# shichaoy/cube_slam

Hardware: AMD Instinct MI355X
Metric: frames/sec front-end (ORB extract + LSD+LBD lines + cuboid: Canny+DT+sweep+score+select) @640x480 (higher is better)
Workload: dtype f64

## Files before the change

cube_slam_amd/csrc/frontend.hip:

```cpp
#include "common.h"

#include <condition_variable>
#include <map>
#include <mutex>
#include <thread>
#include <vector>

extern "C" int cs_lsd_run(cs_ctx *ctx, cs_lsd *l, int with_lbd);
void cs_lsd_set_gate(cs_lsd *l, void (*wait)(void *), void (*done)(void *), void *arg);
void cs_lsd_set_shared_gpu(cs_lsd *l, int shared);
extern "C" int cs_orb_run(cs_ctx *ctx, cs_orb *e);
extern "C" int cs_cuboid_batch_run(cs_ctx *ctx, cs_cuboid_batch *b);
extern "C" int cs_cuboid_batch_set_shared_gpu(cs_cuboid_batch *b, int shared);
extern "C" int cs_cuboid_batch_set_lines(cs_ctx *ctx, cs_cuboid_batch *b, const int *line_offsets, const double *lines);
extern "C" int cs_cuboid_batch_n_frames(const cs_cuboid_batch *b);
extern "C" int cs_cuboid_batch_set_gray_device(cs_ctx *ctx, cs_cuboid_batch *b, const uint8_t *d_gray);
extern "C" int cs_cuboid_batch_set_scene(cs_ctx *ctx, cs_cuboid_batch *b, const double *Twc, const int *box_offsets, const double *boxes, const int *line_offsets, const double *lines);
extern "C" int cs_orb_set_frames_device(cs_ctx *ctx, cs_orb *e, const uint8_t *d_gray, int n_frames);
extern "C" int cs_orb_geometry(const cs_orb *e, int *width, int *height, int *max_frames);
extern "C" int cs_lsd_geometry(const cs_lsd *l, int *width, int *height, int *max_frames);
extern "C" int cs_cuboid_batch_geometry(const cs_cuboid_batch *b, int *width, int *height, int *n_frames);
extern "C" int cs_lsd_set_frames_device(cs_ctx *ctx, cs_lsd *l, const uint8_t *d_gray, int n_frames);
extern "C" int cs_orb_read_packed_on(cs_orb *e, void *stream, cs_keypoint *kps, uint8_t *desc, long cap_total, int *first, long *total);
extern "C" int cs_cuboid_batch_read_on(cs_cuboid_batch *b, void *stream, cs_cuboid *out, int *counts, int *status_out);
int cs_lsd_filter_lines_packed(cs_lsd *l, float length_thres, std::vector<int> &offsets, std::vector<double> &lines);

struct cs_frontend;
namespace {
struct LinePacket { std::vector<int> off; std::vector<double> lines; int status = CS_OK; };
struct Gate {
    std::mutex m; std::condition_variable cv;
    bool phased = false;
    long submitted = 0, target = 0, done = 0;
};
struct FrameRing {
    int n_slots = 0, n_frames = 0; size_t bytes = 0;
    hipStream_t copy = nullptr, copy_out = nullptr;
    hipEvent_t step_done = nullptr, cub_done = nullptr, results_out = nullptr; bool results_pending = false, status_read = false; int *h_status = nullptr;
    std::vector<uint8_t *> d;
    std::vector<hipEvent_t> uploaded, used_main, used_line;
    std::vector<long> main_gen, line_gen;
    struct Scene { bool has = false, has_lines = false; std::vector<double> Twc, boxes, lines; std::vector<int> box_off, line_off; };
    std::vector<Scene> scene;
    std::mutex m; std::condition_variable cv;
    long pushed = 0, first = 0, first_line = 0;
};
struct LineWorker {
    cs_ctx *ctx = nullptr; cs_lsd *lsd = nullptr;
    Gate *gate = nullptr; long ticket = 0; bool marked = true;
    static void gate_wait(void *arg) {
        LineWorker *w = (LineWorker *)arg; Gate *g = w->gate;
        std::unique_lock<std::mutex> lk(g->m);
        if (w->marked) return;
// ... 82 lines not shown
    bool may_start() const { return passes_started < passes_target && passes_started < step_no + lead_max() && (!ring || passes_started < ring->pushed); }
    void kick_idle() {
        for (size_t k = 0; k < workers.size() && may_start(); k++) {
            const size_t c = (next_worker + k) % workers.size();
            if (!workers[c]->is_free()) continue;
            workers[c]->submit(passes_started++);
            next_worker = (c + 1) % workers.size();
        }
    }
};

namespace {
int LineWorker::take_frames() {
    if (!fe || !fe->ring) return CS_OK;
    FrameRing *R = fe->ring;
    const int slot = (int)(pass_no % R->n_slots);
    if (hipSetDevice(ctx->device) != hipSuccess || hipStreamWaitEvent(ctx->stream, R->uploaded[slot], 0) != hipSuccess) return CS_ERR_HIP;
    int r = cs_lsd_set_frames_device(ctx, lsd, R->d[slot], R->n_frames);
    if (r == CS_OK && hipEventRecord(R->used_line[slot], ctx->stream) != hipSuccess) r = CS_ERR_HIP;
    { std::lock_guard<std::mutex> lk(R->m); R->line_gen[slot] = pass_no; }
    R->cv.notify_all();
    return r;
}
bool LineWorker::after_pass(int r) {
    if (!fe) return false;
    LinePacket pk; bool leave = false;
    if (fe->chain && pass_no >= fe->chain_first) {
        leave = true; pk.status = r;
        if (r == CS_OK) pk.status = cs_lsd_filter_lines_packed(lsd, fe->chain_thres, pk.off, pk.lines);
    }
    std::lock_guard<std::mutex> lk(fe->any_m);
    if (leave) { fe->packets[pass_no] = std::move(pk); fe->any_cv.notify_all(); }
    if (r != CS_OK || fe->gate.phased || !fe->may_start()) return false;
    pass_no = fe->passes_started++;
    return true;
}
}

extern "C" {

int cs_frontend_create(cs_ctx *ctx, cs_orb *orb, cs_cuboid_batch *batch, int n_line_workers, cs_ctx *const *line_ctx, cs_lsd *const *lsd, cs_frontend **out) {
    if (!ctx || !out || n_line_workers < 0 || n_line_workers > 8 || (n_line_workers && (!line_ctx || !lsd))) return CS_ERR_BAD_ARG;
    for (int i = 0; i < n_line_workers; i++) if (!line_ctx[i] || !lsd[i] || line_ctx[i] == ctx) return CS_ERR_BAD_ARG;
    cs_frontend *fe = new (std::nothrow) cs_frontend();
    if (!fe) return CS_ERR_NOMEM;
    fe->ctx = ctx; fe->orb = orb; fe->batch = batch;
    for (int i = 0; i < n_line_workers; i++) {
        LineWorker *w = new LineWorker();
        w->ctx = line_ctx[i]; w->lsd = lsd[i]; w->gate = &fe->gate; w->any_m = &fe->any_m; w->any_cv = &fe->any_cv; w->fe = fe;
        cs_lsd_set_gate(w->lsd, LineWorker::gate_wait, LineWorker::gate_done, w);
        w->th = std::thread([w] { w->loop(); });
        fe->workers.push_back(w);
    }
    fe->streams = 1 + 2 * n_line_workers;
    { const char *q = getenv("GPU_MAX_HW_QUEUES"); fe->hw_queues = q && atoi(q) > 0 ? atoi(q) : 4; }
    if (fe->hw_queues < fe->streams) {
        static bool said = false;
        if (!said) { said = true; fprintf(stderr, "[cubeslam-hip] cs_frontend_create: %d streams on %d hardware queues (GPU_MAX_HW_QUEUES%s): streams that share a queue run one after the other -- a 100 ms region walk then "
                                          "stalls another stream's kernels (up to -25 %% measured).  Export GPU_MAX_HW_QUEUES=16 before the HIP runtime starts (INTEGRATION.md).\n", fe->streams, fe->hw_queues, getenv("GPU_MAX_HW_QUEUES") ? "" : " unset: the runtime's default"); }
    }
    if (fe->batch) cs_cuboid_batch_set_shared_gpu(fe->batch, n_line_workers > 0);
    for (LineWorker *w : fe->workers) cs_lsd_set_shared_gpu(w->lsd, n_line_workers > 1);
    *out = fe;
    return CS_OK;
}

int cs_frontend_queues(const cs_frontend *fe, int *streams, int *hw_queues) {
    if (!fe) return CS_ERR_BAD_ARG;
    if (streams) *streams = fe->streams;
    if (hw_queues) *hw_queues = fe->hw_queues;
    return fe->hw_queues >= fe->streams ? 1 : 0;
}

int cs_frontend_step(cs_frontend *fe) {
    if (!fe) return CS_ERR_BAD_ARG;
    int r = CS_OK;
    if (fe->ring) {
        std::lock_guard<std::mutex> lk(fe->any_m);
        if (fe->step_no >= fe->ring->pushed) { fe->ctx->err = "cs_frontend_step: the streaming source holds no frames for this step (cs_frontend_stream_push first)"; return CS_ERR_BAD_ARG; }
    }
    if (!fe->workers.empty()) {
        const long W = (long)fe->workers.size();
        LinePacket pk; bool have_pk = false;
        {
            std::unique_lock<std::mutex> lk(fe->any_m);
            const long k = fe->step_no;
            if (fe->passes_target < k + 1) fe->passes_target = k + 1;
            if (fe->gate.phased) {
                if (fe->passes_started <= k) { LineWorker *w = fe->workers[(size_t)(k % W)]; const long no = fe->passes_started++; lk.unlock(); w->submit(no); lk.lock(); fe->in_phase++; }
            } else {
                fe->kick_idle();
                while (fe->passes_started <= k) { fe->any_cv.wait_for(lk, std::chrono::milliseconds(2)); fe->kick_idle(); }
            }
            if (fe->chain && fe->batch && k - W >= fe->chain_first) {
                fe->any_cv.wait(lk, [&] { return fe->packets.count(k - W) != 0; });
                pk = std::move(fe->packets[k - W]); fe->packets.erase(k - W); have_pk = true;
            }
            fe->step_no = k + 1;
        }
        if (have_pk) {
            r = pk.status;
            if (r == CS_OK && (long)pk.off.size() != (long)cs_cuboid_batch_n_frames(fe->batch) + 1) r = CS_ERR_BAD_ARG;
            if (r == CS_OK) r = cs_cuboid_batch_set_lines(fe->cub_ctx ? fe->cub_ctx : fe->ctx, fe->batch, pk.off.data(), pk.lines.data());
            if (r != CS_OK) return r;
        }
    } else {
        std::lock_guard<std::mutex> lk(fe->any_m);
// ... 203 lines not shown
```

cube_slam_amd/csrc/lsd_regions.h:

```cpp
#pragma once
#include <vector>

#include <hip/hip_runtime.h>
struct cs_ctx;
struct LsdSeq;
int lsd_seq_run(cs_ctx *ctx, LsdSeq **handle, int F, int w, int h, const float *d_ang, const double *d_mod, const int *d_caddr, const float *d_cdeg, const float2 *d_ccs, const int *frame_base,
                std::vector<std::vector<float>> &lines, long *stats, void (*before_seq)(void *), void (*after_seq)(void *), void *gate_arg, int grp_p, int waves_per_workgroup = 16, void *scratch = nullptr,
                size_t scratch_bytes = 0, bool pix_ready = false, bool walk_bg = false);
void lsd_seq_destroy(LsdSeq *r);
```

cube_slam_amd/csrc/lsd_regions.hip:

```cpp
#include "common.h"

#include <cfloat>
#include <climits>
#include <cmath>
#include <vector>

#include "lsd_regions.h"
#include "lsd_rg_seq.h"
#include "lsd_rg_wlk.h"

namespace {
constexpr int PAD_PX = 272, PAD_LIST = 272, PAD_RECT = 34;
constexpr double PI_ = rg::PI_, LOG_EPS = 0.0, LSD_SCALE = 0.8;
struct AngMap { int w, h; const float *deg; };

__device__ __forceinline__ double rg_log_gamma_windschitl(double x) { return 0.918938533204673 + (x - 0.5) * log(x) - x + 0.5 * x * log(x * sinh(1 / x) + 1 / (810.0 * pow(x, 6.0))); }
__device__ double rg_log_gamma(double x) {
    if (x > 15.0) return rg_log_gamma_windschitl(x);
    const double q[7] = {75122.6331530, 80916.6278952, 36308.2951477, 8687.24529705, 1168.92649479, 83.8676043424, 2.50662827511};
    double a = (x + 0.5) * log(x + 5.5) - (x + 5.5), b = 0;
    for (int n = 0; n < 7; ++n) { a -= log(x + double(n)); b += q[n] * pow(x, double(n)); }
    return a + log(b);
}
#ifndef RG_IMPROVE_WAVES
// ... 121 lines not shown
    if (log_nfa > LOG_EPS) return log_nfa;
    const int g = lane >> 3, sub = lane & 7;
    rg::Rect mine;
    int tot = 0, al = 0, cnt = 0;
    auto tolerances = [&]() {
        mine = rec;
        double p = rec.p, precs[5];
#pragma unroll
        for (int n = 0; n < 5; ++n) { p /= 2; precs[n] = p * PI_; if (n <= g) { mine.p = p; mine.prec = precs[n]; } }
        int t, alg[5]; rg_rect_count<5>(F, rec, precs, lane, t, alg);
        tot = t; al = alg[0];
#pragma unroll
        for (int n = 1; n < 5; ++n) if (g == n) al = alg[n];
        cnt = 5;
    };
    auto shrink = [&](int side) {
        mine = rec; cnt = 0;
        double wd = rec.width;
#pragma unroll
        for (int n = 0; n < 5; ++n) if ((wd - delta) >= 0.5) { wd -= delta; cnt++; }
#pragma unroll
        for (int n = 0; n < 5; ++n) if (n <= g && (mine.width - delta) >= 0.5) {
            if (side == 1) { mine.x1 += -mine.dy * delta_2; mine.y1 += mine.dx * delta_2; mine.x2 += -mine.dy * delta_2; mine.y2 += mine.dx * delta_2; }
            else if (side == 2) { mine.x1 -= -mine.dy * delta_2; mine.y1 -= mine.dx * delta_2; mine.x2 -= -mine.dy * delta_2; mine.y2 -= mine.dx * delta_2; }
            mine.width -= delta;
        }
        if (cnt) rg_rect_count_group(F, mine, g < cnt, sub, tot, al);
    };
    auto take_best = [&]() {
        const bool on = g < cnt;
        const double mv = rg_nfa(on ? tot : 0, on ? al : 0, mine.p, LOG_NT, lgt);
        int best = -1;
#pragma unroll
        for (int n = 0; n < 5; ++n) { const double vn = __shfl(mv, 8 * n); if (n < cnt && vn > log_nfa) { log_nfa = vn; best = n; } }
        if (best >= 0) rec = rg_rect_shfl(mine, 8 * best);
    };
    tolerances(); take_best();
    if (log_nfa > LOG_EPS) return log_nfa;
    for (int side = 0; side < 3; side++) {
        shrink(side);
        if (cnt) take_best();
        if (log_nfa > LOG_EPS) return log_nfa;
    }
    if ((rec.width - delta) >= 0.5) { tolerances(); take_best(); }
    return log_nfa;
}

struct SeqParams {
    int F, w, h;
    const int *caddr; const int *frame_base; const float *cdeg; const float2 *ccs; const double *mod; const float *ang;
    float *ang32; float *seed_cs; int *glist; double *rect; size_t rect_stride; int cand_cap; int *cand_cnt; int *status;
    int min_reg_size, list_cap;
    size_t pix_stride;
};
__global__ void __launch_bounds__(256) lsd_rg_fill32(float4 *ang, size_t n4) {
    const size_t i = (size_t)blockIdx.x * 256 + threadIdx.x;
    if (i < n4) ang[i] = make_float4(rgs::NOTDEF_F, rgs::NOTDEF_F, rgs::NOTDEF_F, rgs::NOTDEF_F);
}
__global__ void __launch_bounds__(256) lsd_rg_scatter(SeqParams P) {
    const int f = blockIdx.y, base = P.frame_base[f], ne = P.frame_base[f + 1] - base;
    const int i = blockIdx.x * 256 + threadIdx.x;
    if (i >= ne) return;
    const int q = P.caddr[base + i] & 0x7fffffff;
    const float d = P.cdeg[base + i];
    P.ang32[(size_t)f * P.pix_stride + q] = d;
    const double a = double(d) * rg::DEG_TO_RADS;
    reinterpret_cast<float2 *>(P.seed_cs)[base + i] = make_float2(float(cos(a)), float(sin(a)));
}
__device__ __forceinline__ void lsd_rg_seq_body(const SeqParams &P) {
    const int f = __builtin_amdgcn_readfirstlane(blockIdx.x * (blockDim.x >> 6) + (threadIdx.x >> 6));
    if (f >= P.F) return;
#ifdef RGS_PRIO
    __builtin_amdgcn_s_setprio(RGS_PRIO);
#endif
    const int base = P.frame_base[f];
    rgs::Frame Fr;
    Fr.w = P.w; Fr.h = P.h; Fr.ne = P.frame_base[f + 1] - base;
    Fr.caddr = P.caddr + base; Fr.fre = P.ang32 + (size_t)f * P.pix_stride; Fr.ang = P.ang + (size_t)f * P.w * P.h; Fr.mod = P.mod + (size_t)f * P.w * P.h; Fr.seed_cs = P.seed_cs + 2 * (size_t)base;
    Fr.rect = P.rect + (size_t)f * P.rect_stride; Fr.cand_cap = P.cand_cap; Fr.cand_cnt = P.cand_cnt + f;
    Fr.status = P.status + 4 * f; Fr.min_reg_size = P.min_reg_size; Fr.list_cap = P.list_cap;
    rgs::List L;
    L.glob = P.glist + (size_t)f * rgs::CAP; L.ring[0] = 0;
    rgs::run_frame<rgs::Wave>(Fr, L);
}
#ifdef RGS_WAVES
__global__ void __launch_bounds__(1024) __attribute__((amdgpu_waves_per_eu(RGS_WAVES, RGS_WAVES))) lsd_rg_seq(SeqParams P) { lsd_rg_seq_body(P); }
#else
__global__ void __launch_bounds__(1024) lsd_rg_seq(SeqParams P) { lsd_rg_seq_body(P); }
#endif
constexpr int WLK_SLICES = 8;
struct WlkLaunch { rgl::Batch slice[WLK_SLICES]; int n_slices, waves_per_slice; };
template <int NS> struct WlkMail {
    rgw::Mail<NS> &m; int base;
    __device__ __forceinline__ rgw::Mail<NS> &mail() { return m; }
    __device__ __forceinline__ int slot_of(int l) const { return base + l; }
    __device__ __forceinline__ int ring_size() const { return NS; }
    __device__ __forceinline__ void after_iteration(const rgl::Batch &) {}
};
template <int WK, int NWAVES, int ACC> __global__ void __launch_bounds__(64 * NWAVES) lsd_rg_wlk(WlkLaunch L, int blocks_per_slice) {
    constexpr int NS = WK * 64;
    __shared__ rgw::Mail<NS> mail;
    for (int k = threadIdx.x; k < NS; k += 64 * NWAVES) { mail.slot[k].state = 0; mail.slot[k].fl = 0; mail.ring_id[k] = 0; mail.ring_tick[k] = 0; }
    if (threadIdx.x == 0) { mail.tail = 0; mail.head = 0; mail.walkers_done = 0; }
    __syncthreads();
    const int wv = __builtin_amdgcn_readfirstlane(threadIdx.x >> 6), lane = threadIdx.x & 63;
    const int c = blockIdx.x / blocks_per_slice;
    const rgl::Batch &B = L.slice[c];
    if (wv < WK) {
        const int f0 = ((blockIdx.x - c * blocks_per_slice) * WK + wv) * 64;
        if (f0 < B.F) { WlkMail<NS> mp{mail, wv * 64}; rgw::run_walker<rgl::LWave, ACC>(B, f0, mp); }
        rgw::wg_release();
        if (lane == 0) rgw::lds_add(&mail.walkers_done, 1);
        return;
    }
    for (;;) {
        int t = 0;
        if (lane == 0) t = rgw::lds_add(&mail.head, 1);
        t = __builtin_amdgcn_readfirstlane(t);
        bool quit = false;
        while (__builtin_amdgcn_readfirstlane(rgw::lds_ld(&mail.ring_tick[t % NS])) != t + 1) {
            if (__builtin_amdgcn_readfirstlane(rgw::lds_ld(&mail.walkers_done)) == WK && __builtin_amdgcn_readfirstlane(rgw::lds_ld(&mail.tail)) <= t) { quit = true; break; }
            __builtin_amdgcn_s_sleep(4);
        }
        if (quit) break;
        rgw::serve_ticket<rgs::Wave, NS>(B, mail, t);
    }
}
__global__ void __launch_bounds__(1024) lsd_rg_cand_scan(const int *cand_cnt, int F, int *cand_base) {
    __shared__ int part[1024];
    const int t = threadIdx.x, per = (F + 1023) / 1024;
    int sum = 0;
    for (int k = 0; k < per; k++) { const int f = t * per + k; if (f < F) sum += cand_cnt[f]; }
    part[t] = sum;
    __syncthreads();
    for (int d = 1; d < 1024; d <<= 1) { const int v = t >= d ? part[t - d] : 0; __syncthreads(); part[t] += v; __syncthreads(); }
    int run = part[t] - sum;
    for (int k = 0; k < per; k++) { const int f = t * per + k; if (f < F) { cand_base[f] = run; run += cand_cnt[f]; } }
    if (t == 1023) cand_base[F] = part[1023];
}
__global__ void __launch_bounds__(256) __attribute__((amdgpu_waves_per_eu(RG_IMPROVE_WAVES, RG_IMPROVE_WAVES))) lsd_rg_improve(SeqParams P, const int *cand_base, int n_cand, const double *lgt, float4 *line, uint8_t *has) {
    const int base = (blockIdx.x * 4 + (threadIdx.x >> 6)) * 8, lane = threadIdx.x & 63, grp = lane >> 3, sub = lane & 7;
    if (base >= n_cand) return;
    const double LOG_NT = 5 * (log10(double(P.w)) + log10(double(P.h))) / 2 + log10(11.0);
    auto frame_of = [&](int wv) { int lo = 0, hi = P.F; while (hi - lo > 1) { const int mid = (lo + hi) >> 1; if (cand_base[mid] <= wv) lo = mid; else hi = mid; } return lo; };
    auto load_rect = [&](int wv, int f, rg::Rect &rec) {
        const double *o = P.rect + (size_t)f * P.rect_stride + (size_t)(wv - cand_base[f]) * 12;
        rec.x1 = o[0]; rec.y1 = o[1]; rec.x2 = o[2]; rec.y2 = o[3]; rec.width = o[4]; rec.x = o[5]; rec.y = o[6]; rec.theta = o[7]; rec.dx = o[8]; rec.dy = o[9]; rec.prec = o[10]; rec.p = o[11];
    };
    auto emit = [&](int wv, rg::Rect rec, double log_nfa) {
        const bool ok = log_nfa > LOG_EPS;
        if (ok) {
            rec.x1 += 0.5; rec.y1 += 0.5; rec.x2 += 0.5; rec.y2 += 0.5;
            rec.x1 /= LSD_SCALE; rec.y1 /= LSD_SCALE; rec.x2 /= LSD_SCALE; rec.y2 /= LSD_SCALE;
            line[wv] = make_float4(float(rec.x1), float(rec.y1), float(rec.x2), float(rec.y2));
        }
        has[wv] = ok ? 1 : 0;
    };
    const int mine = base + grp;
    const bool on = mine < n_cand;
    const int f1 = frame_of(on ? mine : n_cand - 1);
    rg::Rect r1;
    load_rect(on ? mine : n_cand - 1, f1, r1);
    double log1;
    {
        RectSpan S; S.set(r1, P.h);
        const float *deg = P.ang + (size_t)f1 * P.w * P.h;
        int tot = 0, alg[1] = {0};
        if (on)
            for (int y = S.y_first + sub; y <= S.y_hi; y += 8) {
                int lx, rx;
                if (!S.row(y, P.w, lx, rx)) continue;
                tot += rx - lx + 1;
                rg_row_count<1>(deg + (size_t)y * P.w, lx, rx, 0, 1, r1.theta, &r1.prec, alg);
            }
        for (int off = 1; off < 8; off <<= 1) { tot += __shfl_xor(tot, off); alg[0] += __shfl_xor(alg[0], off); }
        log1 = rg_nfa(tot, alg[0], r1.p, LOG_NT, lgt);
    }
    if (on && sub == 0 && log1 > LOG_EPS) emit(mine, r1, log1);
    unsigned long long todo = __ballot(on && sub == 0 && !(log1 > LOG_EPS));
    while (todo) {
        const int l = __ffsll((long long)todo) - 1;
        todo &= todo - 1;
        const int wv = base + (l >> 3), f = __shfl(f1, l);
        const double first = __shfl(log1, l);
        rg::Rect rec;
        load_rect(wv, f, rec);
        const AngMap Fr = {P.w, P.h, P.ang + (size_t)f * P.w * P.h};
        const double log_nfa = rg_rect_improve(Fr, rec, LOG_NT, lane, lgt, first);
        if (lane == 0) emit(wv, rec, log_nfa);
    }
}
}

struct LsdSeq {
    int F = 0, w = 0, h = 0; int cand_cap = 0; size_t cap_lines = 0;
    float *d_pix = nullptr; bool pix_borrowed = false;
    rgl::Ent *d_elist = nullptr; float *d_ang32 = nullptr; int *d_order = nullptr;
    int *d_glist = nullptr, *d_cand_cnt = nullptr, *d_cand_base = nullptr, *d_status = nullptr, *d_frame_base = nullptr;
    double *d_rect = nullptr, *d_lgt = nullptr;
    uint8_t *d_has = nullptr;
    float4 *d_line = nullptr;
    cs_pinned<int> h_base, h_status; cs_pinned<uint8_t> h_has; cs_pinned<float4> h_line;
};
void lsd_seq_destroy(LsdSeq *r) {
    if (!r) return;
    void *ptrs[] = {r->d_elist, r->d_ang32, r->d_order, r->pix_borrowed ? nullptr : r->d_pix, r->d_glist, r->d_cand_cnt, r->d_cand_base, r->d_status, r->d_frame_base, r->d_rect, r->d_lgt, r->d_has, r->d_line};
    for (void *p : ptrs) if (p) hipFree(p);
    r->h_base.release(); r->h_status.release(); r->h_has.release(); r->h_line.release();
    delete r;
}
int lsd_seq_run(cs_ctx *ctx, LsdSeq **handle, int F, int w, int h, const float *d_ang, const double *d_mod, const int *d_caddr, const float *d_cdeg, const float2 *d_ccs, const int *frame_base,
                std::vector<std::vector<float>> &lines, long *stats ,
                void (*before_seq)(void *), void (*after_seq)(void *), void *gate_arg ,
                int grp_p ,
                int waves_per_workgroup ,
                void *scratch, size_t scratch_bytes ,
                bool pix_ready ,
                bool walk_bg ) {
    LsdSeq *r = *handle;
    if (w > 0xffff || h > 0x7fff) return CS_ERR_CAPACITY;
    int max_ne = 0;
    for (int f = 0; f < F; f++) max_ne = std::max(max_ne, frame_base[f + 1] - frame_base[f]);
    int rc;
#define RA_(call) do { rc = (call); if (rc != CS_OK) return rc; } while (0)
    if (!r || r->F < F || r->w != w || r->h != h) {
        lsd_seq_destroy(r);
        r = new LsdSeq();
        *handle = r;
        r->F = F; r->w = w; r->h = h; r->cand_cap = 4096;
        RA_(cs_dalloc(ctx, &r->d_order, (size_t)F)); RA_(cs_dalloc(ctx, &r->d_rect, (size_t)F * (r->cand_cap * 12 + PAD_RECT)));
        RA_(cs_dalloc(ctx, &r->d_cand_cnt, (size_t)F)); RA_(cs_dalloc(ctx, &r->d_cand_base, (size_t)F + 1));
        RA_(cs_dalloc(ctx, &r->d_status, (size_t)F * 4)); RA_(cs_dalloc(ctx, &r->d_frame_base, (size_t)F + 1));
        RA_(cs_dalloc(ctx, &r->d_lgt, (size_t)LG_N));
        CS_LAUNCH(ctx, "lsd_rg_lgamma_table", lsd_rg_lgamma_table, dim3(LG_N / 256), dim3(256), 0, r->d_lgt);
    }
    RA_(cs_h2d(ctx, r->d_frame_base, frame_base, (size_t)F + 1));
    SeqParams S;
    S.F = F; S.w = w; S.h = h; S.caddr = d_caddr; S.frame_base = r->d_frame_base; S.cdeg = d_cdeg; S.ccs = d_ccs; S.mod = d_mod; S.ang = d_ang;
    S.ang32 = nullptr; S.seed_cs = reinterpret_cast<float *>(const_cast<float2 *>(d_ccs));  S.glist = r->d_glist; S.rect = r->d_rect; S.cand_cap = r->cand_cap; S.cand_cnt = r->d_cand_cnt; S.status = r->d_status;
    const double LOG_NT = 5 * (std::log10(double(w)) + std::log10(double(h))) / 2 + std::log10(11.0);
    S.min_reg_size = int(-LOG_NT / std::log10(rg::ANG_TH / 180));
    S.list_cap = rgs::CAP;
    if (const char *e = getenv("CUBESLAM_LSD_SEQ_CAP")) S.list_cap = std::max(2, std::min(rgs::CAP, atoi(e)));
    if (grp_p != 0 && grp_p != 65) return CS_ERR_BAD_ARG;
    const bool grp = grp_p == 65, pad = grp;
    const size_t rect_stride = (size_t)r->cand_cap * 12 + (pad ? PAD_RECT : 0), list_stride = (size_t)rgl::CAP + (pad ? PAD_LIST : 0);
    S.pix_stride = (size_t)w * h + (pad ? PAD_PX : 0); S.rect_stride = rect_stride;
    const size_t npx = (size_t)F * S.pix_stride;
    if (grp) {
        const size_t head = (size_t)((w + 8 + 3) & ~3);
        if (!r->d_ang32) RA_(cs_dalloc(ctx, &r->d_ang32, head + (size_t)r->F * ((size_t)w * h + PAD_PX) + 16));
        if (!r->d_elist) RA_(cs_dalloc(ctx, &r->d_elist, (size_t)r->F * ((size_t)rgl::CAP + PAD_LIST) + 16));
        S.ang32 = r->d_ang32 + head;
        CS_LAUNCH(ctx, "lsd_rg_fill", lsd_rg_fill32, dim3((unsigned)(((npx + head) / 4 + 1 + 255) / 256)), dim3(256), 0, reinterpret_cast<float4 *>(r->d_ang32), (npx + head) / 4 + 1);
    } else {
        if (!r->d_pix) {
            if (scratch && scratch_bytes >= (size_t)r->F * w * h * sizeof(float) + 64) { r->d_pix = static_cast<float *>(scratch); r->pix_borrowed = true; }
            else RA_(cs_dalloc(ctx, &r->d_pix, (size_t)r->F * w * h + 16));
        }
        if (!r->d_glist) RA_(cs_dalloc(ctx, &r->d_glist, (size_t)r->F * rgs::CAP));
        S.ang32 = r->d_pix; S.glist = r->d_glist;
        if (pix_ready && !r->pix_borrowed) { ctx->err = "lsd_seq_run: the pixel records were announced in the scratch buffer, but the stage does not use it for this batch"; return CS_ERR_BAD_ARG; }
        if (!pix_ready) CS_LAUNCH(ctx, "lsd_rg_fill", lsd_rg_fill32, dim3((unsigned)((npx / 4 + 1 + 255) / 256)), dim3(256), 0, reinterpret_cast<float4 *>(r->d_pix), npx / 4 + 1);
    }
    if (!pix_ready) CS_LAUNCH(ctx, "lsd_rg_scatter", lsd_rg_scatter, dim3((max_ne + 255) / 256, F), dim3(256), 0, S);
    int wpb = std::max(1, std::min(16, waves_per_workgroup));
    if (before_seq) before_seq(gate_arg);
    if (grp) {
        const size_t npx = (size_t)w * h, head = (size_t)((w + 8 + 3) & ~3);
        int chunk = (int)std::min<size_t>(4096, 0xffffffffull / (npx * sizeof(double)));
        chunk = std::min(chunk, 1024);
        if (chunk < 1) return CS_ERR_CAPACITY;
        std::vector<int> order((size_t)F);
        for (int c0 = 0; c0 < F; c0 += chunk) {
            const int fc = std::min(chunk, F - c0);
            for (int k = 0; k < fc; k++) order[(size_t)c0 + k] = k;
            std::stable_sort(order.begin() + c0, order.begin() + c0 + fc, [&](int a, int b) { return frame_base[c0 + a + 1] - frame_base[c0 + a] > frame_base[c0 + b + 1] - frame_base[c0 + b]; });
        }
        RA_(cs_h2d(ctx, r->d_order, order.data(), (size_t)F));
        CS_HIP(ctx, hipStreamSynchronize(ctx->stream));
        for (int l0 = 0; l0 < F; l0 += chunk * WLK_SLICES) {
            WlkLaunch L;
            L.n_slices = 0; L.waves_per_slice = (chunk + 63) / 64;
            for (int c0 = l0; c0 < F && L.n_slices < WLK_SLICES; c0 += chunk) {
                const int fc = std::min(chunk, F - c0);
                rgl::Batch &B = L.slice[L.n_slices++];
                B.F = fc; B.w = w; B.h = h; B.npx = (int)npx; B.order = r->d_order + c0; B.ang_stride = (int)S.pix_stride; B.list_stride = (int)list_stride; B.rect_stride = (int)rect_stride; B.ang_head = (int)head;
                B.caddr = d_caddr + frame_base[c0]; B.frame_base = r->d_frame_base + c0; B.ang = r->d_ang32 + (size_t)c0 * S.pix_stride; B.mod = d_mod + (size_t)c0 * npx; B.seed_cs = S.seed_cs + 2 * (size_t)frame_base[c0];
                B.list = r->d_elist + (size_t)c0 * list_stride; B.list_cap = std::min(S.list_cap, rgl::CAP); B.rect = r->d_rect + (size_t)c0 * rect_stride; B.cand_cap = r->cand_cap; B.cand_cnt = r->d_cand_cnt + c0; B.status = r->d_status + 4 * (size_t)c0;
                B.min_reg_size = S.min_reg_size; B.max_iters = (int)std::min<size_t>(64 * npx, 0x7fffffff);
            }
            int wk = 1, nw = 8, acc = 1;
            if (const char *e = getenv("CUBESLAM_LSD_WLK")) sscanf(e, "%d,%d,%d", &wk, &nw, &acc);
            const int bps = (L.waves_per_slice + wk - 1) / wk, groups = L.n_slices * bps;
#define WLK_(WK, NW, AC) else if (wk == WK && nw == NW && acc == AC) CS_LAUNCH(ctx, "lsd_rg_wlk", (lsd_rg_wlk<WK, NW, AC>), dim3(groups), dim3(64 * NW), 0, L, bps)
            if (false) {}
            WLK_(1, 8, 1); WLK_(1, 8, 2); WLK_(2, 8, 1); WLK_(8, 16, 1);
            else { ctx->err = "CUBESLAM_LSD_WLK: no such shape (walkers,waves,accepts)"; return CS_ERR_BAD_ARG; }
#undef WLK_
        }
    } else if (walk_bg) {
        CS_HIP(ctx, ctx->bg_begin());
        cs_ctx::pending_ev pe;
        if (ctx->timing) { pe.name = "lsd_rg_seq"; pe.a = ctx->get_event(); pe.b = ctx->get_event(); hipEventRecord(pe.a, ctx->bg_stream); }
        hipLaunchKernelGGL(lsd_rg_seq, dim3((F + wpb - 1) / wpb), dim3(64 * wpb), 0, ctx->bg_stream, S);
        if (ctx->timing) { hipEventRecord(pe.b, ctx->bg_stream); ctx->pending.push_back(pe); }
        CS_HIP(ctx, ctx->bg_end());
    } else
    CS_LAUNCH(ctx, "lsd_rg_seq", lsd_rg_seq, dim3((F + wpb - 1) / wpb), dim3(64 * wpb), 0, S);
    CS_LAUNCH(ctx, "lsd_rg_cand_scan", lsd_rg_cand_scan, dim3(1), dim3(1024), 0, r->d_cand_cnt, F, r->d_cand_base);
    RA_(r->h_base.reserve(ctx, (size_t)F + 1)); RA_(r->h_status.reserve(ctx, (size_t)F * 4));
    RA_(cs_d2h(ctx, r->h_base.p, r->d_cand_base, (size_t)F + 1));
    RA_(cs_d2h(ctx, r->h_status.p, r->d_status, (size_t)F * 4));
    CS_HIP(ctx, hipStreamSynchronize(ctx->stream));
    if (after_seq) after_seq(gate_arg);
    long grows = 0, fetches = 0, nreg = 0;
    bool bad = false;
    for (int f = 0; f < F; f++) { grows += r->h_status.p[4 * f]; bad = bad || r->h_status.p[4 * f + 1] != 0; nreg += r->h_status.p[4 * f + 2]; fetches += r->h_status.p[4 * f + 3]; }
    const int n_cand = r->h_base.p[F];
    if (stats) { stats[0] = grows; stats[1] = fetches; stats[2] = n_cand; stats[3] = nreg; }
    if (bad) return CS_ERR_CAPACITY;
    lines.assign((size_t)F, {});
    if (n_cand == 0) return CS_OK;
    if ((size_t)n_cand > r->cap_lines) {
        if (r->d_line) hipFree(r->d_line); if (r->d_has) hipFree(r->d_has);
        r->d_line = nullptr; r->d_has = nullptr; r->cap_lines = 0;
        const size_t cap = (size_t)n_cand + n_cand / 4 + 1024;
        RA_(cs_dalloc(ctx, &r->d_line, cap)); RA_(cs_dalloc(ctx, &r->d_has, cap));
        r->cap_lines = cap;
    }
    CS_LAUNCH(ctx, "lsd_rg_improve", lsd_rg_improve, dim3((n_cand + 31) / 32), dim3(256), 0, S, r->d_cand_base, n_cand, r->d_lgt, r->d_line, r->d_has);
    RA_(r->h_has.reserve(ctx, (size_t)n_cand)); RA_(r->h_line.reserve(ctx, (size_t)n_cand));
    RA_(cs_d2h(ctx, r->h_has.p, r->d_has, (size_t)n_cand));
    RA_(cs_d2h(ctx, r->h_line.p, r->d_line, (size_t)n_cand));
    CS_HIP(ctx, hipStreamSynchronize(ctx->stream));
#undef RA_
#pragma omp parallel for schedule(static) num_threads(std::max(1, std::min(ctx->host_threads, F)))
    for (int f = 0; f < F; f++)
        for (int k = r->h_base.p[f]; k < r->h_base.p[f + 1]; k++)
            if (r->h_has.p[k]) { const float4 v = r->h_line.p[k]; lines[f].push_back(v.x); lines[f].push_back(v.y); lines[f].push_back(v.z); lines[f].push_back(v.w); }
    return CS_OK;
}
```

Before: 24550.

## Split LSD region walk into frame groups pipelined with rectangle improve

Frames are sorted by candidate-pixel count and split into two groups. Each group's region-growing walk and candidate scan runs on its own stream, so the rectangle-improve kernel, the device-to-host copies and the host assembly of one group overlap with work on the next. The improve kernel now uses 64-thread blocks that take work from an atomic ticket cursor instead of a static grid, and result buffers are grown lazily with a retry pass if they overflow. This adds extra streams and hardware queue pressure, more synchronisation events, and considerable complexity.

Result: slower. 21420 (-12.7%).

```diff
diff --git a/cube_slam_amd/csrc/frontend.hip b/cube_slam_amd/csrc/frontend.hip
--- a/cube_slam_amd/csrc/frontend.hip
+++ b/cube_slam_amd/csrc/frontend.hip
@@ -1,4 +1,5 @@
 #include "common.h"
+#include "lsd_regions.h"
 
 #include <condition_variable>
 #include <map>
@@ -187,7 +188,7 @@
         w->th = std::thread([w] { w->loop(); });
         fe->workers.push_back(w);
     }
-    fe->streams = 1 + 2 * n_line_workers;
+    fe->streams = 1 + (1 + LSD_WALK_GROUPS) * n_line_workers;
     { const char *q = getenv("GPU_MAX_HW_QUEUES"); fe->hw_queues = q && atoi(q) > 0 ? atoi(q) : 4; }
     if (fe->hw_queues < fe->streams) {
         static bool said = false;
diff --git a/cube_slam_amd/csrc/lsd_regions.h b/cube_slam_amd/csrc/lsd_regions.h
--- a/cube_slam_amd/csrc/lsd_regions.h
+++ b/cube_slam_amd/csrc/lsd_regions.h
@@ -4,6 +4,7 @@
 #include <hip/hip_runtime.h>
 struct cs_ctx;
 struct LsdSeq;
+constexpr int LSD_WALK_GROUPS = 2;
 int lsd_seq_run(cs_ctx *ctx, LsdSeq **handle, int F, int w, int h, const float *d_ang, const double *d_mod, const int *d_caddr, const float *d_cdeg, const float2 *d_ccs, const int *frame_base,
                 std::vector<std::vector<float>> &lines, long *stats, void (*before_seq)(void *), void (*after_seq)(void *), void *gate_arg, int grp_p, int waves_per_workgroup = 16, void *scratch = nullptr,
                 size_t scratch_bytes = 0, bool pix_ready = false, bool walk_bg = false);
diff --git a/cube_slam_amd/csrc/lsd_regions.hip b/cube_slam_amd/csrc/lsd_regions.hip
--- a/cube_slam_amd/csrc/lsd_regions.hip
+++ b/cube_slam_amd/csrc/lsd_regions.hip
@@ -197,6 +197,7 @@
     float *ang32; float *seed_cs; int *glist; double *rect; size_t rect_stride; int cand_cap; int *cand_cnt; int *status;
     int min_reg_size, list_cap;
     size_t pix_stride;
+    const int *order;
 };
 __global__ void __launch_bounds__(256) lsd_rg_fill32(float4 *ang, size_t n4) {
     const size_t i = (size_t)blockIdx.x * 256 + threadIdx.x;
@@ -213,8 +214,9 @@
     reinterpret_cast<float2 *>(P.seed_cs)[base + i] = make_float2(float(cos(a)), float(sin(a)));
 }
 __device__ __forceinline__ void lsd_rg_seq_body(const SeqParams &P) {
-    const int f = __builtin_amdgcn_readfirstlane(blockIdx.x * (blockDim.x >> 6) + (threadIdx.x >> 6));
-    if (f >= P.F) return;
+    const int k = __builtin_amdgcn_readfirstlane(blockIdx.x * (blockDim.x >> 6) + (threadIdx.x >> 6));
+    if (k >= P.F) return;
+    const int f = __builtin_amdgcn_readfirstlane(P.order[k]);
 #ifdef RGS_PRIO
     __builtin_amdgcn_s_setprio(RGS_PRIO);
 #endif
@@ -271,25 +273,31 @@
         rgw::serve_ticket<rgs::Wave, NS>(B, mail, t);
     }
 }
-__global__ void __launch_bounds__(1024) lsd_rg_cand_scan(const int *cand_cnt, int F, int *cand_base) {
+__global__ void __launch_bounds__(1024) lsd_rg_cand_scan(const int *cand_cnt, const int *order, int F, int *cand_base, int *total) {
     __shared__ int part[1024];
     const int t = threadIdx.x, per = (F + 1023) / 1024;
+    auto cnt = [&](int k) { return cand_cnt[order ? order[k] : k]; };
     int sum = 0;
-    for (int k = 0; k < per; k++) { const int f = t * per + k; if (f < F) sum += cand_cnt[f]; }
+    for (int k = 0; k < per; k++) { const int f = t * per + k; if (f < F) sum += cnt(f); }
     part[t] = sum;
     __syncthreads();
     for (int d = 1; d < 1024; d <<= 1) { const int v = t >= d ? part[t - d] : 0; __syncthreads(); part[t] += v; __syncthreads(); }
     int run = part[t] - sum;
-    for (int k = 0; k < per; k++) { const int f = t * per + k; if (f < F) { cand_base[f] = run; run += cand_cnt[f]; } }
-    if (t == 1023) cand_base[F] = part[1023];
-}
-__global__ void __launch_bounds__(256) __attribute__((amdgpu_waves_per_eu(RG_IMPROVE_WAVES, RG_IMPROVE_WAVES))) lsd_rg_improve(SeqParams P, const int *cand_base, int n_cand, const double *lgt, float4 *line, uint8_t *has) {
-    const int base = (blockIdx.x * 4 + (threadIdx.x >> 6)) * 8, lane = threadIdx.x & 63, grp = lane >> 3, sub = lane & 7;
-    if (base >= n_cand) return;
+    for (int k = 0; k < per; k++) { const int f = t * per + k; if (f < F) { cand_base[f] = run; run += cnt(f); } }
+    if (t == 1023) { cand_base[F] = part[1023]; *total = part[1023]; }
+}
+__global__ void __launch_bounds__(64) __attribute__((amdgpu_waves_per_eu(RG_IMPROVE_WAVES, RG_IMPROVE_WAVES))) lsd_rg_improve(SeqParams P, const int *cand_base, const int *grp_n, int g, int *cursor, int *flag, int cap,
+                                                                                                                             const double *lgt, float4 *line, uint8_t *has) {
+    const int lane = threadIdx.x, grp = lane >> 3, sub = lane & 7;
+    int off = 0;
+    for (int j = 0; j < g; j++) off += grp_n[j];
+    const int n_cand = grp_n[g];
+    if (off + n_cand > cap) { if (blockIdx.x == 0 && lane == 0) *flag = 1; return; }
+    line += off; has += off;
     const double LOG_NT = 5 * (log10(double(P.w)) + log10(double(P.h))) / 2 + log10(11.0);
     auto frame_of = [&](int wv) { int lo = 0, hi = P.F; while (hi - lo > 1) { const int mid = (lo + hi) >> 1; if (cand_base[mid] <= wv) lo = mid; else hi = mid; } return lo; };
-    auto load_rect = [&](int wv, int f, rg::Rect &rec) {
-        const double *o = P.rect + (size_t)f * P.rect_stride + (size_t)(wv - cand_base[f]) * 12;
+    auto load_rect = [&](int wv, int k, int f, rg::Rect &rec) {
+        const double *o = P.rect + (size_t)f * P.rect_stride + (size_t)(wv - cand_base[k]) * 12;
         rec.x1 = o[0]; rec.y1 = o[1]; rec.x2 = o[2]; rec.y2 = o[3]; rec.width = o[4]; rec.x = o[5]; rec.y = o[6]; rec.theta = o[7]; rec.dx = o[8]; rec.dy = o[9]; rec.prec = o[10]; rec.p = o[11];
     };
     auto emit = [&](int wv, rg::Rect rec, double log_nfa) {
@@ -301,38 +309,44 @@
         }
         has[wv] = ok ? 1 : 0;
     };
-    const int mine = base + grp;
-    const bool on = mine < n_cand;
-    const int f1 = frame_of(on ? mine : n_cand - 1);
-    rg::Rect r1;
-    load_rect(on ? mine : n_cand - 1, f1, r1);
-    double log1;
-    {
-        RectSpan S; S.set(r1, P.h);
-        const float *deg = P.ang + (size_t)f1 * P.w * P.h;
-        int tot = 0, alg[1] = {0};
-        if (on)
-            for (int y = S.y_first + sub; y <= S.y_hi; y += 8) {
-                int lx, rx;
-                if (!S.row(y, P.w, lx, rx)) continue;
-                tot += rx - lx + 1;
-                rg_row_count<1>(deg + (size_t)y * P.w, lx, rx, 0, 1, r1.theta, &r1.prec, alg);
-            }
-        for (int off = 1; off < 8; off <<= 1) { tot += __shfl_xor(tot, off); alg[0] += __shfl_xor(alg[0], off); }
-        log1 = rg_nfa(tot, alg[0], r1.p, LOG_NT, lgt);
-    }
-    if (on && sub == 0 && log1 > LOG_EPS) emit(mine, r1, log1);
-    unsigned long long todo = __ballot(on && sub == 0 && !(log1 > LOG_EPS));
-    while (todo) {
-        const int l = __ffsll((long long)todo) - 1;
-        todo &= todo - 1;
-        const int wv = base + (l >> 3), f = __shfl(f1, l);
-        const double first = __shfl(log1, l);
-        rg::Rect rec;
-        load_rect(wv, f, rec);
-        const AngMap Fr = {P.w, P.h, P.ang + (size_t)f * P.w * P.h};
-        const double log_nfa = rg_rect_improve(Fr, rec, LOG_NT, lane, lgt, first);
-        if (lane == 0) emit(wv, rec, log_nfa);
+    for (;;) {
+        int ticket = 0;
+        if (lane == 0) ticket = atomicAdd(cursor, 1);
+        const int base = __shfl(ticket, 0) * 8;
+        if (base >= n_cand) break;
+        const int mine = base + grp;
+        const bool on = mine < n_cand;
+        const int k1 = frame_of(on ? mine : n_cand - 1), f1 = P.order ? P.order[k1] : k1;
+        rg::Rect r1;
+        load_rect(on ? mine : n_cand - 1, k1, f1, r1);
+        double log1;
+        {
+            RectSpan S; S.set(r1, P.h);
+            const float *deg = P.ang + (size_t)f1 * P.w * P.h;
+            int tot = 0, alg[1] = {0};
+            if (on)
+                for (int y = S.y_first + sub; y <= S.y_hi; y += 8) {
+                    int lx, rx;
+                    if (!S.row(y, P.w, lx, rx)) continue;
+                    tot += rx - lx + 1;
+                    rg_row_count<1>(deg + (size_t)y * P.w, lx, rx, 0, 1, r1.theta, &r1.prec, alg);
+                }
+            for (int off = 1; off < 8; off <<= 1) { tot += __shfl_xor(tot, off); alg[0] += __shfl_xor(alg[0], off); }
+            log1 = rg_nfa(tot, alg[0], r1.p, LOG_NT, lgt);
+        }
+        if (on && sub == 0 && log1 > LOG_EPS) emit(mine, r1, log1);
+        unsigned long long todo = __ballot(on && sub == 0 && !(log1 > LOG_EPS));
+        while (todo) {
+            const int l = __ffsll((long long)todo) - 1;
+            todo &= todo - 1;
+            const int wv = base + (l >> 3), k = __shfl(k1, l), f = __shfl(f1, l);
+            const double first = __shfl(log1, l);
+            rg::Rect rec;
+            load_rect(wv, k, f, rec);
+            const AngMap Fr = {P.w, P.h, P.ang + (size_t)f * P.w * P.h};
+            const double log_nfa = rg_rect_improve(Fr, rec, LOG_NT, lane, lgt, first);
+            if (lane == 0) emit(wv, rec, log_nfa);
+        }
     }
 }
 }
@@ -342,16 +356,20 @@
     float *d_pix = nullptr; bool pix_borrowed = false;
     rgl::Ent *d_elist = nullptr; float *d_ang32 = nullptr; int *d_order = nullptr;
     int *d_glist = nullptr, *d_cand_cnt = nullptr, *d_cand_base = nullptr, *d_status = nullptr, *d_frame_base = nullptr;
+    int *d_grp = nullptr;
+    hipStream_t xs[LSD_WALK_GROUPS] = {}; hipEvent_t ev[LSD_WALK_GROUPS] = {};
     double *d_rect = nullptr, *d_lgt = nullptr;
     uint8_t *d_has = nullptr;
     float4 *d_line = nullptr;
-    cs_pinned<int> h_base, h_status; cs_pinned<uint8_t> h_has; cs_pinned<float4> h_line;
+    cs_pinned<int> h_base, h_status, h_order, h_grp; cs_pinned<uint8_t> h_has; cs_pinned<float4> h_line;
 };
 void lsd_seq_destroy(LsdSeq *r) {
     if (!r) return;
-    void *ptrs[] = {r->d_elist, r->d_ang32, r->d_order, r->pix_borrowed ? nullptr : r->d_pix, r->d_glist, r->d_cand_cnt, r->d_cand_base, r->d_status, r->d_frame_base, r->d_rect, r->d_lgt, r->d_has, r->d_line};
+    for (hipStream_t st : r->xs) if (st) { hipStreamSynchronize(st); hipStreamDestroy(st); }
+    for (hipEvent_t e : r->ev) if (e) hipEventDestroy(e);
+    void *ptrs[] = {r->d_elist, r->d_ang32, r->d_order, r->pix_borrowed ? nullptr : r->d_pix, r->d_glist, r->d_cand_cnt, r->d_cand_base, r->d_status, r->d_frame_base, r->d_rect, r->d_lgt, r->d_has, r->d_line, r->d_grp};
     for (void *p : ptrs) if (p) hipFree(p);
-    r->h_base.release(); r->h_status.release(); r->h_has.release(); r->h_line.release();
+    r->h_base.release(); r->h_status.release(); r->h_order.release(); r->h_grp.release(); r->h_has.release(); r->h_line.release();
     delete r;
 }
 int lsd_seq_run(cs_ctx *ctx, LsdSeq **handle, int F, int w, int h, const float *d_ang, const double *d_mod, const int *d_caddr, const float *d_cdeg, const float2 *d_ccs, const int *frame_base,
@@ -374,7 +392,7 @@
         *handle = r;
         r->F = F; r->w = w; r->h = h; r->cand_cap = 4096;
         RA_(cs_dalloc(ctx, &r->d_order, (size_t)F)); RA_(cs_dalloc(ctx, &r->d_rect, (size_t)F * (r->cand_cap * 12 + PAD_RECT)));
-        RA_(cs_dalloc(ctx, &r->d_cand_cnt, (size_t)F)); RA_(cs_dalloc(ctx, &r->d_cand_base, (size_t)F + 1));
+        RA_(cs_dalloc(ctx, &r->d_cand_cnt, (size_t)F)); RA_(cs_dalloc(ctx, &r->d_cand_base, (size_t)F + LSD_WALK_GROUPS)); RA_(cs_dalloc(ctx, &r->d_grp, (size_t)3 * LSD_WALK_GROUPS));
         RA_(cs_dalloc(ctx, &r->d_status, (size_t)F * 4)); RA_(cs_dalloc(ctx, &r->d_frame_base, (size_t)F + 1));
         RA_(cs_dalloc(ctx, &r->d_lgt, (size_t)LG_N));
         CS_LAUNCH(ctx, "lsd_rg_lgamma_table", lsd_rg_lgamma_table, dim3(LG_N / 256), dim3(256), 0, r->d_lgt);
@@ -382,7 +400,7 @@
     RA_(cs_h2d(ctx, r->d_frame_base, frame_base, (size_t)F + 1));
     SeqParams S;
     S.F = F; S.w = w; S.h = h; S.caddr = d_caddr; S.frame_base = r->d_frame_base; S.cdeg = d_cdeg; S.ccs = d_ccs; S.mod = d_mod; S.ang = d_ang;
-    S.ang32 = nullptr; S.seed_cs = reinterpret_cast<float *>(const_cast<float2 *>(d_ccs));  S.glist = r->d_glist; S.rect = r->d_rect; S.cand_cap = r->cand_cap; S.cand_cnt = r->d_cand_cnt; S.status = r->d_status;
+    S.ang32 = nullptr; S.seed_cs = reinterpret_cast<float *>(const_cast<float2 *>(d_ccs));  S.glist = r->d_glist; S.rect = r->d_rect; S.cand_cap = r->cand_cap; S.cand_cnt = r->d_cand_cnt; S.status = r->d_status; S.order = nullptr;
     const double LOG_NT = 5 * (std::log10(double(w)) + std::log10(double(h))) / 2 + std::log10(11.0);
     S.min_reg_size = int(-LOG_NT / std::log10(rg::ANG_TH / 180));
     S.list_cap = rgs::CAP;
@@ -409,7 +427,52 @@
         if (!pix_ready) CS_LAUNCH(ctx, "lsd_rg_fill", lsd_rg_fill32, dim3((unsigned)((npx / 4 + 1 + 255) / 256)), dim3(256), 0, reinterpret_cast<float4 *>(r->d_pix), npx / 4 + 1);
     }
     if (!pix_ready) CS_LAUNCH(ctx, "lsd_rg_scatter", lsd_rg_scatter, dim3((max_ne + 255) / 256, F), dim3(256), 0, S);
-    int wpb = std::max(1, std::min(16, waves_per_workgroup));
+    const int wpb = std::max(1, std::min(16, waves_per_workgroup));
+    const int G = grp ? 1 : std::min(LSD_WALK_GROUPS, F);
+    int gs[LSD_WALK_GROUPS + 1], off[LSD_WALK_GROUPS + 1] = {0};
+    for (int g = 0; g <= G; g++) gs[g] = (int)((long)g * F / G);
+    RA_(r->h_order.reserve(ctx, (size_t)F)); RA_(r->h_base.reserve(ctx, (size_t)F + G)); RA_(r->h_status.reserve(ctx, (size_t)F * 4)); RA_(r->h_grp.reserve(ctx, 3 * LSD_WALK_GROUPS));
+    if (r->cap_lines) { RA_(r->h_has.reserve(ctx, r->cap_lines)); RA_(r->h_line.reserve(ctx, r->cap_lines)); }
+    int *const order = r->h_order.p;
+    if (!grp) {
+        for (int f = 0; f < F; f++) order[f] = f;
+        std::stable_sort(order, order + F, [&](int a, int b) { return frame_base[a + 1] - frame_base[a] < frame_base[b + 1] - frame_base[b]; });
+        RA_(cs_h2d(ctx, r->d_order, order, (size_t)F));
+    } else
+        for (int f = 0; f < F; f++) order[f] = f;
+    int *const d_grp_n = r->d_grp, *const d_cursor = r->d_grp + LSD_WALK_GROUPS, *const d_flag = r->d_grp + 2 * LSD_WALK_GROUPS;
+    CS_HIP(ctx, hipMemsetAsync(r->d_grp, 0, 3 * LSD_WALK_GROUPS * sizeof(int), ctx->stream));
+    auto group_params = [&](int g) { SeqParams Sg = S; Sg.F = gs[g + 1] - gs[g]; Sg.order = grp ? nullptr : r->d_order + gs[g]; return Sg; };
+    auto timed = [&](const char *name, hipStream_t st, auto &&launch) {
+        cs_ctx::pending_ev pe;
+        if (ctx->timing) { pe.name = name; pe.a = ctx->get_event(); pe.b = ctx->get_event(); hipEventRecord(pe.a, st); }
+        launch();
+        if (ctx->timing) { hipEventRecord(pe.b, st); ctx->pending.push_back(pe); }
+    };
+    auto walk = [&](int g, hipStream_t st) {
+        const SeqParams Sg = group_params(g);
+        timed("lsd_rg_seq", st, [&] { hipLaunchKernelGGL(lsd_rg_seq, dim3((Sg.F + wpb - 1) / wpb), dim3(64 * wpb), 0, st, Sg); });
+    };
+    auto scan = [&](int g, hipStream_t st) {
+        timed("lsd_rg_cand_scan", st, [&] { hipLaunchKernelGGL(lsd_rg_cand_scan, dim3(1), dim3(1024), 0, st, r->d_cand_cnt, grp ? (const int *)nullptr : r->d_order + gs[g], gs[g + 1] - gs[g], r->d_cand_base + gs[g] + g, d_grp_n + g); });
+    };
+    auto improve = [&](int g) {
+        const SeqParams Sg = group_params(g);
+        const int waves = (int)std::min<long>(256 * 4 * RG_IMPROVE_WAVES, std::max<long>(1, (long)Sg.F * r->cand_cap / 8));
+        CS_LAUNCH(ctx, "lsd_rg_improve", lsd_rg_improve, dim3(waves), dim3(64), 0, Sg, r->d_cand_base + gs[g] + g, d_grp_n, g, d_cursor + g, d_flag + g, (int)std::min<size_t>(r->cap_lines, INT_MAX), r->d_lgt, r->d_line, r->d_has);
+    };
+    lines.assign((size_t)F, {});
+    auto assemble = [&](int g) {
+        const int *base = r->h_base.p + gs[g] + g, n = gs[g + 1] - gs[g];
+        const uint8_t *has = r->h_has.p + off[g]; const float4 *line = r->h_line.p + off[g];
+#pragma omp parallel for schedule(static) num_threads(std::max(1, std::min(ctx->host_threads, n)))
+        for (int k = 0; k < n; k++) {
+            std::vector<float> &out = lines[(size_t)order[gs[g] + k]];
+            out.clear();
+            for (int i = base[k]; i < base[k + 1]; i++)
+                if (has[i]) { const float4 v = line[i]; out.push_back(v.x); out.push_back(v.y); out.push_back(v.z); out.push_back(v.w); }
+        }
+    };
     if (before_seq) before_seq(gate_arg);
     if (grp) {
         const size_t npx = (size_t)w * h, head = (size_t)((w + 8 + 3) & ~3);
@@ -445,44 +508,81 @@
 #undef WLK_
         }
     } else if (walk_bg) {
+        if (!r->ev[0]) {
+            int lo = 0, hi = 0;
+            const bool prio = hipDeviceGetStreamPriorityRange(&lo, &hi) == hipSuccess && lo != hi;
+            for (int g = 0; g < LSD_WALK_GROUPS; g++) CS_HIP(ctx, hipEventCreateWithFlags(&r->ev[g], hipEventDisableTiming));
+            for (int g = 0; g + 1 < LSD_WALK_GROUPS; g++) CS_HIP(ctx, prio ? hipStreamCreateWithPriority(&r->xs[g], hipStreamNonBlocking, lo) : hipStreamCreateWithFlags(&r->xs[g], hipStreamNonBlocking));
+        }
         CS_HIP(ctx, ctx->bg_begin());
-        cs_ctx::pending_ev pe;
-        if (ctx->timing) { pe.name = "lsd_rg_seq"; pe.a = ctx->get_event(); pe.b = ctx->get_event(); hipEventRecord(pe.a, ctx->bg_stream); }
-        hipLaunchKernelGGL(lsd_rg_seq, dim3((F + wpb - 1) / wpb), dim3(64 * wpb), 0, ctx->bg_stream, S);
-        if (ctx->timing) { hipEventRecord(pe.b, ctx->bg_stream); ctx->pending.push_back(pe); }
-        CS_HIP(ctx, ctx->bg_end());
-    } else
-    CS_LAUNCH(ctx, "lsd_rg_seq", lsd_rg_seq, dim3((F + wpb - 1) / wpb), dim3(64 * wpb), 0, S);
-    CS_LAUNCH(ctx, "lsd_rg_cand_scan", lsd_rg_cand_scan, dim3(1), dim3(1024), 0, r->d_cand_cnt, F, r->d_cand_base);
-    RA_(r->h_base.reserve(ctx, (size_t)F + 1)); RA_(r->h_status.reserve(ctx, (size_t)F * 4));
-    RA_(cs_d2h(ctx, r->h_base.p, r->d_cand_base, (size_t)F + 1));
+        for (int g = 0; g < G; g++) {
+            const hipStream_t st = g == G - 1 ? ctx->bg_stream : r->xs[g];
+            if (st != ctx->bg_stream) CS_HIP(ctx, hipStreamWaitEvent(st, ctx->bg_in, 0));
+            walk(g, st); scan(g, st);
+            CS_HIP(ctx, hipEventRecord(r->ev[g], st));
+        }
+    }
+    hipEvent_t copied[LSD_WALK_GROUPS] = {};
+    bool outgrown = false;
+    auto finish = [&](int g) -> int {
+        if (!copied[g]) return CS_OK;
+        CS_HIP(ctx, hipEventSynchronize(copied[g]));
+        ctx->pool.push_back(copied[g]); copied[g] = nullptr;
+        assemble(g);
+        return CS_OK;
+    };
+    for (int g = 0; g < G; g++) {
+        const int n = gs[g + 1] - gs[g];
+        if (!grp && walk_bg) CS_HIP(ctx, hipStreamWaitEvent(ctx->stream, r->ev[g], 0));
+        else { if (!grp) walk(g, ctx->stream); scan(g, ctx->stream); }
+        RA_(cs_d2h(ctx, r->h_base.p + gs[g] + g, r->d_cand_base + gs[g] + g, (size_t)n + 1));
+        hipEvent_t counted = ctx->get_event();
+        CS_HIP(ctx, hipEventRecord(counted, ctx->stream));
+        improve(g);
+        if (g > 0) RA_(finish(g - 1));
+        CS_HIP(ctx, hipEventSynchronize(counted));
+        ctx->pool.push_back(counted);
+        const int n_g = r->h_base.p[gs[g] + g + n];
+        off[g + 1] = off[g] + n_g;
+        if ((size_t)off[g + 1] > r->cap_lines) outgrown = true;
+        else if (n_g > 0) {
+            RA_(cs_d2h(ctx, r->h_has.p + off[g], r->d_has + off[g], (size_t)n_g));
+            RA_(cs_d2h(ctx, r->h_line.p + off[g], r->d_line + off[g], (size_t)n_g));
+            copied[g] = ctx->get_event();
+            CS_HIP(ctx, hipEventRecord(copied[g], ctx->stream));
+        }
+    }
+    if (after_seq) after_seq(gate_arg);
     RA_(cs_d2h(ctx, r->h_status.p, r->d_status, (size_t)F * 4));
+    RA_(cs_d2h(ctx, r->h_grp.p, r->d_grp, (size_t)3 * LSD_WALK_GROUPS));
     CS_HIP(ctx, hipStreamSynchronize(ctx->stream));
-    if (after_seq) after_seq(gate_arg);
+    RA_(finish(G - 1));
     long grows = 0, fetches = 0, nreg = 0;
-    bool bad = false;
+    bool bad = false, flagged = false;
     for (int f = 0; f < F; f++) { grows += r->h_status.p[4 * f]; bad = bad || r->h_status.p[4 * f + 1] != 0; nreg += r->h_status.p[4 * f + 2]; fetches += r->h_status.p[4 * f + 3]; }
-    const int n_cand = r->h_base.p[F];
+    for (int g = 0; g < G; g++) flagged = flagged || r->h_grp.p[2 * LSD_WALK_GROUPS + g] != 0;
+    const int n_cand = off[G];
     if (stats) { stats[0] = grows; stats[1] = fetches; stats[2] = n_cand; stats[3] = nreg; }
     if (bad) return CS_ERR_CAPACITY;
-    lines.assign((size_t)F, {});
-    if (n_cand == 0) return CS_OK;
-    if ((size_t)n_cand > r->cap_lines) {
+    if (flagged != outgrown) { ctx->err = "lsd_seq_run: the rectangle kernel and the host disagree on whether the pass fits its result buffers"; return CS_ERR_HIP; }
+    if (outgrown) {
+        const size_t cap = (size_t)n_cand + n_cand / 4 + 1024;
+        float4 *nl = nullptr; uint8_t *nh = nullptr;
+        RA_(cs_dalloc(ctx, &nl, cap));
+        rc = cs_dalloc(ctx, &nh, cap);
+        if (rc != CS_OK) { hipFree(nl); return rc; }
         if (r->d_line) hipFree(r->d_line); if (r->d_has) hipFree(r->d_has);
-        r->d_line = nullptr; r->d_has = nullptr; r->cap_lines = 0;
-        const size_t cap = (size_t)n_cand + n_cand / 4 + 1024;
-        RA_(cs_dalloc(ctx, &r->d_line, cap)); RA_(cs_dalloc(ctx, &r->d_has, cap));
-        r->cap_lines = cap;
-    }
-    CS_LAUNCH(ctx, "lsd_rg_improve", lsd_rg_improve, dim3((n_cand + 31) / 32), dim3(256), 0, S, r->d_cand_base, n_cand, r->d_lgt, r->d_line, r->d_has);
-    RA_(r->h_has.reserve(ctx, (size_t)n_cand)); RA_(r->h_line.reserve(ctx, (size_t)n_cand));
-    RA_(cs_d2h(ctx, r->h_has.p, r->d_has, (size_t)n_cand));
-    RA_(cs_d2h(ctx, r->h_line.p, r->d_line, (size_t)n_cand));
-    CS_HIP(ctx, hipStreamSynchronize(ctx->stream));
+        r->d_line = nl; r->d_has = nh; r->cap_lines = cap;
+        RA_(r->h_has.reserve(ctx, cap)); RA_(r->h_line.reserve(ctx, cap));
+        CS_HIP(ctx, hipMemsetAsync(d_cursor, 0, 2 * LSD_WALK_GROUPS * sizeof(int), ctx->stream));
+        for (int g = 0; g < G; g++) improve(g);
+        RA_(cs_d2h(ctx, r->h_has.p, r->d_has, (size_t)n_cand));
+        RA_(cs_d2h(ctx, r->h_line.p, r->d_line, (size_t)n_cand));
+        RA_(cs_d2h(ctx, r->h_grp.p, r->d_grp, (size_t)3 * LSD_WALK_GROUPS));
+        CS_HIP(ctx, hipStreamSynchronize(ctx->stream));
+        for (int g = 0; g < G; g++) if (r->h_grp.p[2 * LSD_WALK_GROUPS + g]) { ctx->err = "lsd_seq_run: the rectangle kernel left a group alone after its buffers were grown"; return CS_ERR_HIP; }
+        for (int g = 0; g < G; g++) assemble(g);
+    }
 #undef RA_
-#pragma omp parallel for schedule(static) num_threads(std::max(1, std::min(ctx->host_threads, F)))
-    for (int f = 0; f < F; f++)
-        for (int k = r->h_base.p[f]; k < r->h_base.p[f + 1]; k++)
-            if (r->h_has.p[k]) { const float4 v = r->h_line.p[k]; lines[f].push_back(v.x); lines[f].push_back(v.y); lines[f].push_back(v.z); lines[f].push_back(v.w); }
     return CS_OK;
 }
```
